# CliqueOfficial/zk-dcap-verifier

Hardware: AMD Instinct MI355X
Metric: proofs/hour sgx_dcap_verifier k=19 (create_proof on the GPU: commitments, lookups, grand products, NTTs, evaluate_h, evaluations, SHPLONK, host transcript; witness synthesis excluded) (higher is better)
Workload: dtype u32x8 (256-bit Montgomery integers)

## Files before the change

zk-dcap-verifier_amd/csrc/lookupperm.hip:

```cpp
#include "ctx.h"
#include <vector>

namespace zk {

constexpr uint32_t FS_T = 256, FS_E = 16, FS_TILE = FS_T * FS_E, FS_PAD = 258;

ZK_HD uint32_t fs_digit(uint2 k, uint32_t pass) { return ((pass < 4 ? k.x : k.y) >> (8 * (pass & 3))) & 255u; }

constexpr uint32_t XS_T = 256, XS_E = 8, XS_TILE = XS_T * XS_E;

ZK_HD int lp_cmp(const u256& a, const u256& b) {
    for (int i = 7; i >= 0; i--) {
        if (a.v[i] < b.v[i]) return -1;
        if (a.v[i] > b.v[i]) return 1;
    }
    return 0;
}
static uint32_t lp_scan_threads(uint32_t m) {
    uint32_t t = 64;
    while (t < 1024 && t * 8 < m) t <<= 1;
    return t;
}

struct LpbArgs {
    const void* const* cols;
    void* const* outs;
    const void* const* scols;
    const uint32_t* tabcol;
    uint32_t u, n, nb, S, C, nwg, nxs;
    void* canon; uint2* key_a; uint2* key_b; uint32_t* idx_a; uint32_t* idx_b;
    uint32_t* flags; uint32_t* ranks; uint32_t* leftover; uint32_t* ghist; uint32_t* xsums; uint32_t* scal;
    uint32_t* cscal;
    const uint32_t* shifts;
    const void* blind;
};
ZK_KERNEL void lpb_canon_kernel(LpbArgs a) {
    __shared__ uint32_t lor[8];
    const uint32_t s = blockIdx.y, i = blockIdx.x * blockDim.x + threadIdx.x;
    if (threadIdx.x < 8) lor[threadIdx.x] = 0;
    __syncthreads();
    if (i < a.u) {
        const u256 c = Fr::from_mont(load_u256(a.scols[s], i));
        store_u256(a.canon, (size_t)s * a.u + i, c);
#pragma unroll
        for (int w = 0; w < 8; w++) if (c.v[w] & ~lor[w]) atomicOr(&lor[w], c.v[w]);
    }
    __syncthreads();
    if (threadIdx.x < 8 && lor[threadIdx.x]) atomicOr(&a.cscal[s * 16 + threadIdx.x], lor[threadIdx.x]);
}
ZK_KERNEL void lpb_keys_kernel(LpbArgs a) {
    const uint32_t s = blockIdx.y, i = blockIdx.x * blockDim.x + threadIdx.x;
    if (i >= a.u) return;
    const uint32_t shift = a.shifts[s];
    const uint32_t* w = reinterpret_cast<const uint32_t*>(a.canon) + ((size_t)s * a.u + i) * 8;
    const uint32_t ws = shift >> 5, bs = shift & 31;
    uint32_t x[3];
#pragma unroll
    for (int j = 0; j < 3; j++) x[j] = ws + j < 8 ? w[ws + j] : 0u;
    uint2 k;
    k.x = bs ? (x[0] >> bs) | (x[1] << (32 - bs)) : x[0];
    k.y = bs ? (x[1] >> bs) | (x[2] << (32 - bs)) : x[1];
    a.key_a[(size_t)s * a.u + i] = k;
    a.idx_a[(size_t)s * a.u + i] = i;
}
ZK_KERNEL void lpb_hist_kernel(const uint2* keys, uint32_t u, uint32_t pass, uint32_t* ghist, uint32_t nwg) {
    __shared__ uint32_t lh[256];
    const uint32_t s = blockIdx.y, tid = threadIdx.x, base = blockIdx.x * FS_TILE;
    keys += (size_t)s * u;
    lh[tid] = 0;
    __syncthreads();
    for (uint32_t e = 0; e < FS_E; e++) {
        const uint32_t i = base + e * FS_T + tid;
        bool live = i < u;
        const uint32_t d = live ? fs_digit(keys[i], pass) : 0u;
#ifndef ZK_EMU
#pragma unroll
        for (int round = 0; round < 2; round++) {
            if (live) {
                const uint32_t lead = (uint32_t)__builtin_amdgcn_readfirstlane((int)d);
                const bool same = d == lead;
                const unsigned long long m = __ballot(same);
                if (same) {
                    if ((__lane_id() & 63u) == (uint32_t)__builtin_ctzll(m)) atomicAdd(&lh[lead], (uint32_t)__builtin_popcountll(m));
                    live = false;
                }
            }
        }
#endif
        if (live) atomicAdd(&lh[d], 1u);
    }
    __syncthreads();
    ghist[((size_t)s * nwg + blockIdx.x) * 256 + tid] = lh[tid];
}
ZK_KERNEL void lpb_offsets_kernel(uint32_t* ghist, uint32_t nwg) {
    __shared__ uint32_t scan[256];
    const uint32_t s = blockIdx.x, tid = threadIdx.x;
    uint32_t* h = ghist + (size_t)s * nwg * 256;
    uint32_t total = 0;
    for (uint32_t w = 0; w < nwg; w++) total += h[(size_t)w * 256 + tid];
    scan[tid] = total;
    __syncthreads();
    for (uint32_t d = 1; d < 256; d <<= 1) {
        const uint32_t add = tid >= d ? scan[tid - d] : 0;
        __syncthreads();
        scan[tid] += add;
        __syncthreads();
    }
    uint32_t run = scan[tid] - total;
    for (uint32_t w = 0; w < nwg; w++) {
        const uint32_t c = h[(size_t)w * 256 + tid];
        h[(size_t)w * 256 + tid] = run;
        run += c;
    }
}
ZK_KERNEL void lpb_scatter_kernel(const uint2* keys_in, const uint32_t* idx_in, uint2* keys_out, uint32_t* idx_out, uint32_t u, uint32_t pass,
                                  const uint32_t* gbase_all, uint32_t nwg) {
    __shared__ __attribute__((aligned(16))) uint16_t cnt[FS_T * FS_PAD];
    __shared__ uint32_t gbase[256];
    const uint32_t s = blockIdx.y, tid = threadIdx.x, wg = blockIdx.x, base = wg * FS_TILE;
    keys_in += (size_t)s * u; idx_in += (size_t)s * u; keys_out += (size_t)s * u; idx_out += (size_t)s * u;
    {
        uint4* c4 = reinterpret_cast<uint4*>(cnt);
        constexpr uint32_t n4 = FS_T * FS_PAD * 2 / 16;
        for (uint32_t q = tid; q < n4; q += FS_T) c4[q] = make_uint4(0, 0, 0, 0);
    }
    gbase[tid] = gbase_all[((size_t)s * nwg + wg) * 256 + tid];
    __syncthreads();
    uint2 k[FS_E];
    uint32_t v[FS_E];
    uint16_t rl[FS_E];
    const uint32_t lo = base + tid * FS_E;
#pragma unroll
    for (uint32_t e = 0; e < FS_E; e++) {
        const uint32_t i = lo + e;
        if (i < u) {
            k[e] = keys_in[i]; v[e] = idx_in[i];
            rl[e] = cnt[tid * FS_PAD + fs_digit(k[e], pass)]++;
        }
    }
    __syncthreads();
    {
        uint32_t run = 0;
        for (uint32_t t = 0; t < FS_T; t++) {
            const uint32_t c = cnt[t * FS_PAD + tid];
            cnt[t * FS_PAD + tid] = (uint16_t)run;
            run += c;
        }
    }
    __syncthreads();
#pragma unroll
    for (uint32_t e = 0; e < FS_E; e++) {
        const uint32_t i = lo + e;
        if (i < u) {
            const uint32_t d = fs_digit(k[e], pass);
            const uint32_t pos = gbase[d] + cnt[tid * FS_PAD + d] + rl[e];
            keys_out[pos] = k[e];
            idx_out[pos] = v[e];
        }
    }
}
ZK_KERNEL void lpb_check_kernel(LpbArgs a, const uint32_t* idx_sorted) {
    const uint32_t s = blockIdx.y, i = blockIdx.x * blockDim.x + threadIdx.x;
    if (i == 0 || i >= a.u || a.shifts[s] == 0) return;
    const uint32_t* canon = reinterpret_cast<const uint32_t*>(a.canon) + (size_t)s * a.u * 8;
    const uint32_t* idx = idx_sorted + (size_t)s * a.u;
    const uint32_t* x = canon + (size_t)idx[i - 1] * 8;
    const uint32_t* y = canon + (size_t)idx[i] * 8;
    for (int w = 7; w >= 0; w--) {
        if (x[w] < y[w]) return;
        if (x[w] > y[w]) { atomicAdd(&a.cscal[s * 16 + 8], 1u); return; }
    }
}
ZK_KERNEL void lpb_tiemask_kernel(LpbArgs a, const uint32_t* idx_sorted) {
    __shared__ uint32_t lor[8];
    const uint32_t s = blockIdx.y, i = blockIdx.x * blockDim.x + threadIdx.x;
    if (a.cscal[s * 16 + 8] == 0) return;
    if (threadIdx.x < 8) lor[threadIdx.x] = 0;
    __syncthreads();
    if (i > 0 && i < a.u) {
        const uint32_t shift = a.shifts[s];
        const uint32_t* canon = reinterpret_cast<const uint32_t*>(a.canon) + (size_t)s * a.u * 8;
        const uint32_t* idx = idx_sorted + (size_t)s * a.u;
        const uint32_t* x = canon + (size_t)idx[i - 1] * 8;
        const uint32_t* y = canon + (size_t)idx[i] * 8;
        uint32_t d[8], above = 0;
#pragma unroll
        for (int w = 0; w < 8; w++) {
            d[w] = x[w] ^ y[w];
            const uint32_t lo_bit = (uint32_t)w * 32;
            uint32_t in_window = lo_bit + 32 <= shift ? 0u : (lo_bit >= shift ? 0xffffffffu : (0xffffffffu << (shift - lo_bit)));
            above |= d[w] & in_window;
        }
        if (above == 0) {
#pragma unroll
            for (int w = 0; w < 8; w++) if (d[w] & ~lor[w]) atomicOr(&lor[w], d[w]);
        }
    }
    __syncthreads();
    if (threadIdx.x < 8 && lor[threadIdx.x]) atomicOr(&a.cscal[s * 16 + threadIdx.x], lor[threadIdx.x]);
}
ZK_KERNEL void lpb_rekey_kernel(LpbArgs a, const uint32_t* fcols, const uint32_t* fshift, const uint32_t* idx_in, uint2* key_out, uint32_t* idx_out) {
    const uint32_t f = blockIdx.y, i = blockIdx.x * blockDim.x + threadIdx.x;
    if (i >= a.u) return;
    const uint32_t c = fcols[f], shift = fshift[f];
    const uint32_t r = idx_in ? idx_in[(size_t)f * a.u + i] : i;
    const uint32_t* w = reinterpret_cast<const uint32_t*>(a.canon) + ((size_t)c * a.u + r) * 8;
    const uint32_t ws = shift >> 5, bs = shift & 31;
    uint32_t x[3];
#pragma unroll
    for (int j = 0; j < 3; j++) x[j] = ws + j < 8 ? w[ws + j] : 0u;
    uint2 k;
    k.x = bs ? (x[0] >> bs) | (x[1] << (32 - bs)) : x[0];
    k.y = bs ? (x[1] >> bs) | (x[2] << (32 - bs)) : x[1];
    key_out[(size_t)f * a.u + i] = k;
    idx_out[(size_t)f * a.u + i] = r;
}
ZK_KERNEL void lpb_mark_kernel(LpbArgs a, const uint32_t* idx_sorted) {
    const uint32_t l = blockIdx.y, i = blockIdx.x * blockDim.x + threadIdx.x, u = a.u;
    if (i >= u) return;
    const uint32_t tc = a.tabcol[l];
    const void* in_canon = (const char*)a.canon + (size_t)l * u * 32;
    const void* tab_canon = (const char*)a.canon + (size_t)tc * u * 32;
    const uint32_t* in_idx = idx_sorted + (size_t)l * u;
    const uint32_t* tab_idx = idx_sorted + (size_t)tc * u;
    uint32_t* repeated = a.flags + (size_t)(2 * l) * u;
    uint32_t* unconsumed = a.flags + (size_t)(2 * l + 1) * u;
    const u256 v = load_u256(in_canon, in_idx[i]);
    const bool first = i == 0 || lp_cmp(v, load_u256(in_canon, in_idx[i - 1])) != 0;
    repeated[i] = first ? 0u : 1u;
    if (!first) return;
    uint32_t lo = 0, hi = u;
    while (lo < hi) {
        const uint32_t mid = (lo + hi) >> 1;
        if (lp_cmp(load_u256(tab_canon, tab_idx[mid]), v) < 0) lo = mid + 1; else hi = mid;
    }
    if (lo >= u || lp_cmp(load_u256(tab_canon, tab_idx[lo]), v) != 0) { atomicAdd(&a.scal[l * 16 + 1], 1u); return; }
    unconsumed[lo] = 0;
}
ZK_KERNEL void lpb_fill_unconsumed_kernel(LpbArgs a) {
    const uint32_t l = blockIdx.y, i = blockIdx.x * blockDim.x + threadIdx.x;
    if (i < a.u) a.flags[(size_t)(2 * l + 1) * a.u + i] = 1u;
}
ZK_KERNEL void lpb_tile_sum_kernel(LpbArgs a) {
    __shared__ uint32_t part[XS_T];
    const uint32_t s = blockIdx.y, tid = threadIdx.x, base = blockIdx.x * XS_TILE;
    const uint32_t* v = a.ranks + (size_t)s * a.u;
    uint32_t sum = 0;
    for (uint32_t e = 0; e < XS_E; e++) { const uint32_t i = base + e * XS_T + tid; if (i < a.u) sum += v[i]; }
    part[tid] = sum;
    __syncthreads();
    for (uint32_t d = XS_T >> 1; d > 0; d >>= 1) { if (tid < d) part[tid] += part[tid + d]; __syncthreads(); }
    if (tid == 0) a.xsums[(size_t)s * a.nxs + blockIdx.x] = part[0];
}
ZK_KERNEL void lpb_sum_scan_kernel(LpbArgs a) {
    __shared__ uint32_t part[1024];
    const uint32_t s = blockIdx.x, T = blockDim.x, tid = threadIdx.x, m = a.nxs - 1;
    uint32_t* v = a.xsums + (size_t)s * a.nxs;
    const uint32_t per = (m + T - 1) / T;
    const uint32_t lo = tid * per < m ? tid * per : m, hi = lo + per < m ? lo + per : m;
    uint32_t sum = 0;
    for (uint32_t i = lo; i < hi; i++) sum += v[i];
    part[tid] = sum;
    __syncthreads();
    for (uint32_t d = 1; d < T; d <<= 1) {
        const uint32_t add = tid >= d ? part[tid - d] : 0;
        __syncthreads();
        part[tid] += add;
        __syncthreads();
    }
    uint32_t run = part[tid] - sum;
    for (uint32_t i = lo; i < hi; i++) { const uint32_t x = v[i]; v[i] = run; run += x; }
    if (tid == T - 1) a.scal[(s >> 1) * 16 + 2 + (s & 1)] = part[T - 1];
}
ZK_KERNEL void lpb_apply_kernel(LpbArgs a) {
    __shared__ uint32_t part[XS_T];
    const uint32_t s = blockIdx.y, tid = threadIdx.x, lo = blockIdx.x * XS_TILE + tid * XS_E, m = a.u;
    uint32_t* v = a.ranks + (size_t)s * a.u;
    uint32_t x[XS_E], sum = 0;
#pragma unroll
    for (uint32_t e = 0; e < XS_E; e++) { x[e] = lo + e < m ? v[lo + e] : 0u; sum += x[e]; }
    part[tid] = sum;
    __syncthreads();
    for (uint32_t d = 1; d < XS_T; d <<= 1) {
        const uint32_t add = tid >= d ? part[tid - d] : 0;
        __syncthreads();
        part[tid] += add;
        __syncthreads();
    }
    uint32_t run = a.xsums[(size_t)s * a.nxs + blockIdx.x] + part[tid] - sum;
#pragma unroll
    for (uint32_t e = 0; e < XS_E; e++) { if (lo + e < m) v[lo + e] = run; run += x[e]; }
}
ZK_KERNEL void lpb_compact_kernel(LpbArgs a) {
    const uint32_t l = blockIdx.y, t = blockIdx.x * blockDim.x + threadIdx.x;
    if (t < a.u && a.flags[(size_t)(2 * l + 1) * a.u + t]) a.leftover[(size_t)l * a.u + a.ranks[(size_t)(2 * l + 1) * a.u + t]] = t;
}
ZK_KERNEL void lpb_assemble_kernel(LpbArgs a, const uint32_t* idx_sorted) {
    const uint32_t l = blockIdx.y, i = blockIdx.x * blockDim.x + threadIdx.x, u = a.u;
    if (i >= a.n) return;
    void* out_in = a.outs[2 * l];
    void* out_tab = a.outs[2 * l + 1];
    if (i >= u) {
        store_u256(out_in, i, load_u256(a.blind, (size_t)(2 * l) * a.nb + (i - u)));
        store_u256(out_tab, i, load_u256(a.blind, (size_t)(2 * l + 1) * a.nb + (i - u)));
        return;
    }
    const uint32_t* in_idx = idx_sorted + (size_t)l * u;
    const uint32_t* tab_idx = idx_sorted + (size_t)a.tabcol[l] * u;
    const u256 v = load_u256(a.cols[2 * l], in_idx[i]);
    store_u256(out_in, i, v);
    if (!a.flags[(size_t)(2 * l) * u + i]) store_u256(out_tab, i, v);
    else {
        const uint32_t n_rep = a.scal[l * 16 + 2];
        store_u256(out_tab, i, load_u256(a.cols[2 * l + 1], tab_idx[a.leftover[(size_t)l * u + (n_rep - 1 - a.ranks[(size_t)(2 * l) * u + i])]]));
    }
}

int lookup_permute_batch(zk_ctx* ctx, const void* const* d_inputs, const void* const* d_tables, size_t count, uint32_t k, uint32_t blinding_factors,
                         const void* h_blind_inputs, const void* h_blind_tables, void* const* d_out_inputs, void* const* d_out_tables) {
    if (count == 0) return ZK_OK;
    if (!d_inputs || !d_tables || !d_out_inputs || !d_out_tables || !h_blind_inputs || !h_blind_tables)
        return ctx->fail(ZK_ERR_ARG, "zk_lookup_permute_batch_dev: null argument");
    if (k < 1 || k > 26 || count > 4096) return ctx->fail(ZK_ERR_ARG, "zk_lookup_permute_batch_dev: k = %u / count = %zu out of range", k, count);
    const uint32_t n = 1u << k, nb = blinding_factors + 1;
    if (nb >= n) return ctx->fail(ZK_ERR_ARG, "zk_lookup_permute_batch_dev: blinding_factors too large");
    for (size_t l = 0; l < count; l++)
        if (!d_inputs[l] || !d_tables[l] || !d_out_inputs[l] || !d_out_tables[l]) return ctx->fail(ZK_ERR_ARG, "zk_lookup_permute_batch_dev: null column %zu", l);
    const uint32_t u = n - nb, S = 2 * (uint32_t)count;
    std::vector<const void*> scols(d_inputs, d_inputs + count);
    std::vector<uint32_t> tabcol(count);
    for (size_t l = 0; l < count; l++) {
        size_t c = count;
        while (c < scols.size() && scols[c] != d_tables[l]) c++;
        if (c == scols.size()) scols.push_back(d_tables[l]);
        tabcol[l] = (uint32_t)c;
    }
    const uint32_t C = (uint32_t)scols.size();
    const uint32_t nwg = (u + FS_TILE - 1) / FS_TILE, nxs = (u + XS_TILE - 1) / XS_TILE + 1;
    size_t off = 0;
    auto take = [&](size_t bytes) { size_t o = off; off += (bytes + 255) & ~(size_t)255; return o; };
    const size_t o_canon = take((size_t)C * u * 32), o_blind = take((size_t)S * nb * 32), o_ka = take((size_t)C * u * 8), o_kb = take((size_t)C * u * 8),
                 o_ia = take((size_t)C * u * 4), o_ib = take((size_t)C * u * 4), o_fl = take((size_t)S * u * 4), o_rk = take((size_t)S * u * 4),
                 o_lo = take((size_t)count * u * 4), o_gh = take((size_t)C * nwg * 256 * 4), o_xs = take((size_t)S * nxs * 4), o_sc = take((size_t)count * 64),
                 o_cs = take((size_t)C * 64), o_sh = take((size_t)C * 4), o_tc = take((size_t)count * 4), o_cp = take((size_t)S * sizeof(void*)),
                 o_op = take((size_t)S * sizeof(void*)), o_sp = take((size_t)C * sizeof(void*));
    ZK_HIP(ctx->ws_tmp.ensure(off + 256));
    char* base = (char*)ctx->ws_tmp.p;
    hipStream_t st = ctx->stream;
    std::vector<const void*> cols(S);
    std::vector<void*> outs(S);
    std::vector<unsigned char> blind((size_t)S * nb * 32);
    for (size_t l = 0; l < count; l++) {
        cols[2 * l] = d_inputs[l]; cols[2 * l + 1] = d_tables[l];
        outs[2 * l] = d_out_inputs[l]; outs[2 * l + 1] = d_out_tables[l];
        memcpy(&blind[(2 * l) * (size_t)nb * 32], (const char*)h_blind_inputs + l * (size_t)nb * 32, (size_t)nb * 32);
        memcpy(&blind[(2 * l + 1) * (size_t)nb * 32], (const char*)h_blind_tables + l * (size_t)nb * 32, (size_t)nb * 32);
    }
    ZK_HIP(hipMemcpyAsync(base + o_cp, cols.data(), S * sizeof(void*), hipMemcpyHostToDevice, st));
    ZK_HIP(hipMemcpyAsync(base + o_op, outs.data(), S * sizeof(void*), hipMemcpyHostToDevice, st));
    ZK_HIP(hipMemcpyAsync(base + o_sp, scols.data(), C * sizeof(void*), hipMemcpyHostToDevice, st));
    ZK_HIP(hipMemcpyAsync(base + o_tc, tabcol.data(), count * 4, hipMemcpyHostToDevice, st));
    ZK_HIP(hipMemcpyAsync(base + o_blind, blind.data(), blind.size(), hipMemcpyHostToDevice, st));
    ZK_HIP(hipMemsetAsync(base + o_sc, 0, count * 64, st));
    ZK_HIP(hipMemsetAsync(base + o_cs, 0, (size_t)C * 64, st));
    LpbArgs a;
    memset(&a, 0, sizeof a);
    a.cols = (const void* const*)(base + o_cp); a.outs = (void* const*)(base + o_op); a.scols = (const void* const*)(base + o_sp);
    a.tabcol = (const uint32_t*)(base + o_tc);
    a.u = u; a.n = n; a.nb = nb; a.S = S; a.C = C; a.nwg = nwg; a.nxs = nxs;
    a.canon = base + o_canon; a.key_a = (uint2*)(base + o_ka); a.key_b = (uint2*)(base + o_kb); a.idx_a = (uint32_t*)(base + o_ia); a.idx_b = (uint32_t*)(base + o_ib);
    a.flags = (uint32_t*)(base + o_fl); a.ranks = (uint32_t*)(base + o_rk); a.leftover = (uint32_t*)(base + o_lo); a.ghist = (uint32_t*)(base + o_gh);
    a.xsums = (uint32_t*)(base + o_xs); a.scal = (uint32_t*)(base + o_sc); a.cscal = (uint32_t*)(base + o_cs); a.shifts = (const uint32_t*)(base + o_sh);
    a.blind = base + o_blind;
    const int blk = ctx->tune.vec_block;
    const uint32_t g = (u + blk - 1) / blk;
    ZK_LAUNCH(lpb_canon_kernel, dim3(g, C), blk, 0, st, a);
    ZK_CHECK_LAUNCH();
    std::vector<uint32_t> sc((size_t)count * 16), csc((size_t)C * 16);
    ZK_HIP(hipMemcpyAsync(csc.data(), a.cscal, (size_t)C * 64, hipMemcpyDeviceToHost, st));
    ZK_HIP(hipStreamSynchronize(st));
    std::vector<uint32_t> shifts(C);
    uint32_t max_bits = 1;
    bool any_shift = false;
    for (uint32_t c = 0; c < C; c++) {
        const uint32_t* om = &csc[(size_t)c * 16];
        uint32_t nbits = 1;
        for (int wd = 7; wd >= 0; wd--)
            if (om[wd]) { uint32_t top = 31; while (!((om[wd] >> top) & 1)) top--; nbits = (uint32_t)wd * 32 + top + 1; break; }
        shifts[c] = nbits > 64 ? nbits - 64 : 0;
        any_shift |= shifts[c] != 0;
        max_bits = std::max(max_bits, std::min(nbits, 64u));
    }
    ZK_HIP(hipMemcpyAsync(base + o_sh, shifts.data(), (size_t)C * 4, hipMemcpyHostToDevice, st));
    uint32_t* sorted = a.idx_a;
    const bool use_order_check = any_shift;

    auto compact_sort = [&](const std::vector<uint32_t>& fcols, const std::vector<std::vector<uint32_t>>& stage_shift, const std::vector<uint32_t>& stage_bits) -> int {
        const uint32_t Fn = (uint32_t)fcols.size();
        if (!Fn) return ZK_OK;
        const size_t per = (size_t)Fn * u;
        size_t o2 = 0;
        auto take2 = [&](size_t bytes) { size_t o = o2; o2 += (bytes + 255) & ~(size_t)255; return o; };
        const size_t q_ka = take2(per * 8), q_kb = take2(per * 8), q_ia = take2(per * 4), q_ib = take2(per * 4), q_gh = take2((size_t)Fn * nwg * 256 * 4),
                     q_fc = take2((size_t)Fn * 4), q_fs = take2((size_t)Fn * 4 * stage_shift.size());
        ZK_HIP(ctx->ws_mid.ensure(o2 + 256));
        char* b2 = (char*)ctx->ws_mid.p;
        uint2 *rk_in = (uint2*)(b2 + q_ka), *rk_out = (uint2*)(b2 + q_kb);
        uint32_t *ri_in = (uint32_t*)(b2 + q_ia), *ri_out = (uint32_t*)(b2 + q_ib), *rgh = (uint32_t*)(b2 + q_gh);
        ZK_HIP(hipMemcpyAsync(b2 + q_fc, fcols.data(), (size_t)Fn * 4, hipMemcpyHostToDevice, st));
        for (size_t t = 0; t < stage_shift.size(); t++)
            ZK_HIP(hipMemcpyAsync(b2 + q_fs + t * Fn * 4, stage_shift[t].data(), (size_t)Fn * 4, hipMemcpyHostToDevice, st));
        const uint32_t* order = nullptr;
        for (size_t t = 0; t < stage_shift.size(); t++) {
            ZK_LAUNCH(lpb_rekey_kernel, dim3(g, Fn), blk, 0, st, a, (const uint32_t*)(b2 + q_fc), (const uint32_t*)(b2 + q_fs + t * Fn * 4), order, rk_in, ri_in);
            ZK_CHECK_LAUNCH();
            const uint32_t ps = (stage_bits[t] + 7) / 8;
            for (uint32_t p = 0; p < ps; p++) {
                ZK_LAUNCH(lpb_hist_kernel, dim3(nwg, Fn), FS_T, 0, st, (const uint2*)rk_in, u, p, rgh, nwg);
                ZK_CHECK_LAUNCH();
                ZK_LAUNCH(lpb_offsets_kernel, Fn, 256, 0, st, rgh, nwg);
                ZK_CHECK_LAUNCH();
                ZK_LAUNCH(lpb_scatter_kernel, dim3(nwg, Fn), FS_T, 0, st, (const uint2*)rk_in, (const uint32_t*)ri_in, rk_out, ri_out, u, p, (const uint32_t*)rgh, nwg);
                ZK_CHECK_LAUNCH();
                std::swap(rk_in, rk_out);
                std::swap(ri_in, ri_out);
            }
            std::swap(rk_in, rk_out);
            std::swap(ri_in, ri_out);
            order = ri_out;
        }
        for (uint32_t f = 0; f < Fn; f++)
            ZK_HIP(hipMemcpyAsync(sorted + (size_t)fcols[f] * u, order + (size_t)f * u, (size_t)u * 4, hipMemcpyDeviceToDevice, st));
        return ZK_OK;
    };
    auto low_stages = [&](const std::vector<uint32_t>& fcols, const std::vector<uint32_t>& lo_bit, const std::vector<uint32_t>& hi_bit,
                          std::vector<std::vector<uint32_t>>& stage_shift, std::vector<uint32_t>& stage_bits) {
        const uint32_t Fn = (uint32_t)fcols.size();
        uint32_t n_low = 0;
        for (uint32_t f = 0; f < Fn; f++) if (lo_bit[f] < 256) n_low = std::max(n_low, (hi_bit[f] - lo_bit[f]) / 64 + 1);
        for (uint32_t t = 0; t < n_low; t++) {
            std::vector<uint32_t> sh(Fn);
            uint32_t bits = 1;
            for (uint32_t f = 0; f < Fn; f++) {
                const uint32_t st_lo = lo_bit[f] == 256 ? 256 : lo_bit[f] + 64 * t;
                if (st_lo > hi_bit[f] || st_lo >= 256) { sh[f] = 255; continue; }
                sh[f] = st_lo;
                bits = std::max(bits, std::min(64u, hi_bit[f] - st_lo + 1));
            }
            stage_shift.push_back(sh); stage_bits.push_back(bits);
        }
        std::vector<uint32_t> sh(Fn);
        for (uint32_t f = 0; f < Fn; f++) sh[f] = shifts[fcols[f]];
        stage_shift.push_back(sh); stage_bits.push_back(max_bits);
    };
    auto tie_ranges = [&](const std::vector<uint32_t>& cols_, std::vector<uint32_t>& lo_bit, std::vector<uint32_t>& hi_bit) -> int {
        for (uint32_t c : cols_) ZK_HIP(hipMemsetAsync((char*)a.cscal + (size_t)c * 64, 0, 32, st));
        ZK_LAUNCH(lpb_tiemask_kernel, dim3(g, C), blk, 0, st, a, (const uint32_t*)sorted); ZK_CHECK_LAUNCH();
        ZK_HIP(hipMemcpyAsync(csc.data(), a.cscal, (size_t)C * 64, hipMemcpyDeviceToHost, st));
// ... 92 lines not shown
```

zk-dcap-verifier_amd/csrc/mockprover.hip:

```cpp
#include "ctx.h"
#include "quotient.h"
#include <algorithm>
#include <atomic>
#include <list>
#include <random>
#include <string>

namespace zk {
int quotient_program_load(zk_ctx* ctx, const void* blob, size_t len, uint64_t* prog);
int quotient_program_release(zk_ctx* ctx, uint64_t prog);

namespace {
constexpr uint32_t MP_T = 256, MP_E = 8, MP_TILE = MP_T * MP_E, MP_WAVES = MP_T / 64;
constexpr uint32_t MP_LOCAL = 2 * MP_T;

__device__ inline uint64_t mp_ballot(bool p, uint32_t* lds) {
#ifdef ZK_EMU
    const uint32_t tid = threadIdx.x;
    lds[tid] = p ? 1u : 0u;
    __syncthreads();
    uint64_t m = 0;
    for (uint32_t l = 0; l < 64; l++) if (lds[(tid & ~63u) + l]) m |= 1ull << l;
    __syncthreads();
    return m;
#else
    (void)lds;
    return __ballot(p);
#endif
}

ZK_KERNEL void ZK_LAUNCH_BOUNDS(256) mp_count_kernel(const uint8_t* flags, uint64_t count, uint32_t* tile_counts) {
    __shared__ uint32_t bl[MP_T];
    __shared__ uint32_t wc[MP_WAVES];
    const uint32_t tid = threadIdx.x, wave = tid >> 6, lane = tid & 63u;
    const uint64_t base = (uint64_t)blockIdx.x * MP_TILE;
    uint32_t mine = 0;
    for (uint32_t e = 0; e < MP_E; e++) {
        const uint64_t i = base + (uint64_t)e * MP_T + tid;
        mine += (uint32_t)__builtin_popcountll(mp_ballot(i < count && flags[i], bl));
    }
    if (lane == 0) wc[wave] = mine;
    __syncthreads();
    if (tid == 0) {
        uint32_t s = 0;
        for (uint32_t w = 0; w < MP_WAVES; w++) s += wc[w];
        tile_counts[blockIdx.x] = s;
    }
}
ZK_KERNEL void ZK_LAUNCH_BOUNDS(256) mp_scan_kernel(uint32_t* counts, uint32_t n_tiles) {
    __shared__ uint32_t s[MP_T];
    const uint32_t tid = threadIdx.x, per = (n_tiles + MP_T - 1) / MP_T;
    const uint32_t lo = tid * per < n_tiles ? tid * per : n_tiles, hi = lo + per < n_tiles ? lo + per : n_tiles;
    uint32_t sum = 0;
    for (uint32_t i = lo; i < hi; i++) sum += counts[i];
    s[tid] = sum;
    __syncthreads();
    for (uint32_t d = 1; d < MP_T; d <<= 1) {
        const uint32_t v = tid >= d ? s[tid - d] : 0u;
        __syncthreads();
        s[tid] += v;
        __syncthreads();
    }
    uint32_t run = s[tid] - sum;
    for (uint32_t i = lo; i < hi; i++) { const uint32_t c = counts[i]; counts[i] = run; run += c; }
    if (tid == MP_T - 1) counts[n_tiles] = s[MP_T - 1];
}
ZK_KERNEL void ZK_LAUNCH_BOUNDS(256) mp_scatter_kernel(const uint8_t* flags, uint64_t count, const uint32_t* tile_offsets, uint32_t* out) {
    __shared__ uint32_t bl[MP_T];
    __shared__ uint32_t wc[MP_E][MP_WAVES];
    const uint32_t tid = threadIdx.x, wave = tid >> 6, lane = tid & 63u;
    const uint64_t base = (uint64_t)blockIdx.x * MP_TILE;
    uint64_t masks[MP_E];
    for (uint32_t e = 0; e < MP_E; e++) {
        const uint64_t i = base + (uint64_t)e * MP_T + tid;
        masks[e] = mp_ballot(i < count && flags[i], bl);
        if (lane == 0) wc[e][wave] = (uint32_t)__builtin_popcountll(masks[e]);
    }
    __syncthreads();
    uint32_t pos = tile_offsets[blockIdx.x];
    for (uint32_t e = 0; e < MP_E; e++) {
        uint32_t before = 0;
        for (uint32_t w = 0; w < wave; w++) before += wc[e][w];
        if ((masks[e] >> lane) & 1ull)
            out[pos + before + (uint32_t)__builtin_popcountll(masks[e] & ((1ull << lane) - 1ull))] = (uint32_t)(base + (uint64_t)e * MP_T + tid);
        for (uint32_t w = 0; w < MP_WAVES; w++) pos += wc[e][w];
    }
}

ZK_KERNEL void mp_nonzero_kernel(const void* vals, uint32_t u, uint8_t* flags) {
    const uint32_t i = blockIdx.x * blockDim.x + threadIdx.x;
    if (i < u) flags[i] = Fr::is_zero(load_u256(vals, i)) ? 0 : 1;
}

ZK_HD bool mp_less(const u256& a, const u256& b) {
    for (int w = 7; w >= 0; w--)
        if (a.v[w] != b.v[w]) return a.v[w] < b.v[w];
    return false;
}
ZK_KERNEL void mp_table_init_kernel(const void* src, uint32_t u, uint32_t n, void* dst) {
    const uint32_t i = blockIdx.x * blockDim.x + threadIdx.x;
    if (i >= n) return;
    u256 v;
    if (i < u) v = load_u256(src, i);
    else for (int w = 0; w < 8; w++) v.v[w] = 0xffffffffu;
    store_u256(dst, i, v);
}
ZK_KERNEL void mp_bitonic_step_kernel(void* v, uint32_t n, uint32_t size, uint32_t dist) {
    const uint32_t t = blockIdx.x * blockDim.x + threadIdx.x;
    if (t >= n / 2) return;
    const uint32_t lo = ((t & ~(dist - 1u)) << 1) | (t & (dist - 1u)), hi = lo | dist;
    const u256 a = load_u256(v, lo), b = load_u256(v, hi);
    if (mp_less(b, a) == ((lo & size) == 0)) { store_u256(v, lo, b); store_u256(v, hi, a); }
}
ZK_KERNEL void ZK_LAUNCH_BOUNDS(256) mp_bitonic_local_kernel(void* v, uint32_t size_lo, uint32_t size_hi) {
    __shared__ uint4 s[2 * MP_LOCAL];
    const uint32_t tid = threadIdx.x, T = blockDim.x, base = blockIdx.x * 2 * T;
    const uint4* g = reinterpret_cast<const uint4*>(v) + 2 * (size_t)base;
    for (uint32_t j = tid; j < 4 * T; j += T) s[j] = g[j];
    __syncthreads();
    for (uint32_t size = size_lo; size <= size_hi; size <<= 1) {
        for (uint32_t dist = size / 2 < T ? size / 2 : T; dist > 0; dist >>= 1) {
            const uint32_t lo = ((tid & ~(dist - 1u)) << 1) | (tid & (dist - 1u)), hi = lo | dist;
            u256 a, b;
            const uint4 a0 = s[2 * lo], a1 = s[2 * lo + 1], b0 = s[2 * hi], b1 = s[2 * hi + 1];
            a.v[0] = a0.x; a.v[1] = a0.y; a.v[2] = a0.z; a.v[3] = a0.w; a.v[4] = a1.x; a.v[5] = a1.y; a.v[6] = a1.z; a.v[7] = a1.w;
            b.v[0] = b0.x; b.v[1] = b0.y; b.v[2] = b0.z; b.v[3] = b0.w; b.v[4] = b1.x; b.v[5] = b1.y; b.v[6] = b1.z; b.v[7] = b1.w;
            if (mp_less(b, a) == (((base + lo) & size) == 0)) { s[2 * lo] = b0; s[2 * lo + 1] = b1; s[2 * hi] = a0; s[2 * hi + 1] = a1; }
            __syncthreads();
        }
    }
    uint4* o = reinterpret_cast<uint4*>(v) + 2 * (size_t)base;
    for (uint32_t j = tid; j < 4 * T; j += T) o[j] = s[j];
}
ZK_KERNEL void mp_search_kernel(const void* in, const void* sorted, uint32_t k, uint32_t u, uint8_t* flags) {
    const uint32_t r = blockIdx.x * blockDim.x + threadIdx.x;
    if (r >= u) return;
    const u256 x = load_u256(in, r);
    uint32_t pos = 0;
    for (uint32_t b = (1u << k) >> 1; b; b >>= 1)
        if (mp_less(load_u256(sorted, pos + b - 1), x)) pos += b;
    flags[r] = Fr::eq(load_u256(sorted, pos), x) ? 0 : 1;
}
ZK_KERNEL void mp_copy_kernel(const void* const* cols, const uint32_t* map_c, const uint32_t* map_r, uint32_t n_cols, uint32_t k, uint8_t* flags, uint32_t* bad) {
    const uint64_t e = (uint64_t)blockIdx.x * blockDim.x + threadIdx.x;
    if (e >= ((uint64_t)n_cols << k)) return;
    const uint32_t j = (uint32_t)(e >> k), row = (uint32_t)e & ((1u << k) - 1u), cj = map_c[e], rj = map_r[e];
    uint8_t f = 0;
    if (cj >= n_cols || rj >= (1u << k)) atomicOr(bad, 1u);
    else if (cj != j || rj != row) f = Fr::eq(Fr::normalize(load_u256(cols[j], row)), Fr::normalize(load_u256(cols[cj], rj))) ? 0 : 1;
    flags[e] = f;
}

ZK_KERNEL void ZK_LAUNCH_BOUNDS(256) mp_edge_flag_kernel(const uint32_t* map_c, const uint32_t* map_r, uint32_t n_cols, uint32_t k, uint8_t* flags, uint32_t* bad) {
    const uint64_t cells = (uint64_t)n_cols << k, stride = (uint64_t)gridDim.x * blockDim.x;
    for (uint64_t e = (uint64_t)blockIdx.x * blockDim.x + threadIdx.x; e < cells; e += stride) {
        const uint32_t cj = map_c[e], rj = map_r[e];
        uint8_t f = 0;
        if (cj >= n_cols || rj >= (1u << k)) atomicOr(bad, 1u);
        else f = (((uint64_t)cj << k) | rj) != e ? 1 : 0;
        flags[e] = f;
    }
}
ZK_KERNEL void ZK_LAUNCH_BOUNDS(256) mp_edge_gather_kernel(const uint32_t* moved, uint32_t n_edges, const uint32_t* map_c, const uint32_t* map_r, uint32_t k, uint2* edges) {
    const uint32_t stride = gridDim.x * blockDim.x;
    for (uint64_t i = blockIdx.x * blockDim.x + threadIdx.x; i < n_edges; i += stride) {
        const uint32_t c = moved[i];
        edges[i] = make_uint2(c, (map_c[c] << k) | map_r[c]);
    }
}
ZK_KERNEL void ZK_LAUNCH_BOUNDS(256) mp_copy_edges_kernel(const void* const* cols, const uint2* edges, uint32_t n_edges, uint32_t k, uint8_t* flags) {
    const uint32_t stride = gridDim.x * blockDim.x, mask = (1u << k) - 1u;
    for (uint64_t i = blockIdx.x * blockDim.x + threadIdx.x; i < n_edges; i += stride) {
        const uint2 e = edges[i];
        flags[i] = Fr::eq(Fr::normalize(load_u256(cols[e.x >> k], e.x & mask)), Fr::normalize(load_u256(cols[e.y >> k], e.y & mask))) ? 0 : 1;
    }
}
ZK_KERNEL void ZK_LAUNCH_BOUNDS(256) mp_edge_pick_kernel(const uint32_t* picked, uint32_t count, const uint2* edges, uint2* out) {
    const uint32_t stride = gridDim.x * blockDim.x;
    for (uint64_t i = blockIdx.x * blockDim.x + threadIdx.x; i < count; i += stride) out[i] = edges[picked[i]];
}

struct MpMem {
    std::list<DevTmp> held;
    void* get(size_t bytes) {
        held.emplace_back();
        if (hipMalloc(&held.back().p, bytes ? bytes : 32) != hipSuccess) { held.back().p = nullptr; return nullptr; }
        return held.back().p;
    }
};

int mp_oom(zk_ctx* ctx, const char* fn) { return ctx->fail(ZK_ERR_HIP, "%s: device allocation failed", fn); }

int mp_compact(zk_ctx* ctx, const char* fn, const uint8_t* d_flags, uint64_t count, uint32_t* cnt, DevBuf& list, uint32_t* total) {
    const uint32_t tiles = (uint32_t)((count + MP_TILE - 1) / MP_TILE);
    *total = 0;
    if (!tiles) return ZK_OK;
    ZK_LAUNCH(mp_count_kernel, tiles, MP_T, 0, ctx->stream, d_flags, count, cnt);
    ZK_CHECK_LAUNCH();
    ZK_LAUNCH(mp_scan_kernel, 1, MP_T, 0, ctx->stream, cnt, tiles);
    ZK_CHECK_LAUNCH();
    ZK_HIP(hipMemcpyAsync(total, cnt + tiles, 4, hipMemcpyDeviceToHost, ctx->stream));
    ZK_HIP(hipStreamSynchronize(ctx->stream));
    if (!*total) return ZK_OK;
    if (list.ensure((size_t)*total * 4) != hipSuccess) return mp_oom(ctx, fn);
    ZK_LAUNCH(mp_scatter_kernel, tiles, MP_T, 0, ctx->stream, d_flags, count, (const uint32_t*)cnt, (uint32_t*)list.p);
    ZK_CHECK_LAUNCH();
    return ZK_OK;
}

int mp_sort(zk_ctx* ctx, void* d_v, uint32_t k) {
    const uint32_t n = 1u << k, T = std::min<uint32_t>(MP_T, n / 2), L = 2 * T;
    ZK_LAUNCH(mp_bitonic_local_kernel, n / L, T, 0, ctx->stream, d_v, 2u, L);
    ZK_CHECK_LAUNCH();
    for (uint32_t size = 2 * L; size <= n; size <<= 1) {
        for (uint32_t dist = size / 2; dist >= L; dist >>= 1) {
            ZK_LAUNCH(mp_bitonic_step_kernel, (n / 2 + 255) / 256, 256, 0, ctx->stream, d_v, n, size, dist);
            ZK_CHECK_LAUNCH();
        }
        ZK_LAUNCH(mp_bitonic_local_kernel, n / L, T, 0, ctx->stream, d_v, size, size);
        ZK_CHECK_LAUNCH();
    }
    return ZK_OK;
}

u256 mp_random_nonzero(std::mt19937_64& g) {
    for (;;) {
        u256 x;
        for (int i = 0; i < 8; i += 2) { const uint64_t w = g(); x.v[i] = (uint32_t)w; x.v[i + 1] = (uint32_t)(w >> 32); }
        x.v[7] &= 0x3fffffffu;
        x = Fr::reduce_once(x);
        if (!Fr::is_zero(x)) return x;
    }
}

struct MpTimer {
    EvTimer t;
    MpTimer(zk_ctx* ctx, const char* label) : t(ctx, label) {}
    void done() { t.stop(); t.resolve(); }
};

}

struct MockPlan {
    bool copy_edges;
    bool resident_tables;
};
constexpr MockPlan MP_ONE_SHOT{false, false};
constexpr MockPlan MP_SESSION{true, true};

struct MockSession {
    zk_ctx* ctx;
    MockPlan plan = MP_SESSION;
    uint32_t k = 0, n = 0, u = 0, F = 0, A = 0, I = 0, L = 0, M = 0, n_challenges = 0, n_polys = 0, words = 0, n_edges = 0, n_programs = 0;
    uint64_t cells = 0;
    size_t bytes = 0;
    std::vector<void*> owned;
    std::vector<uint64_t> progs;
    std::vector<uint32_t> perm_cols;
    std::vector<const void*> fx;
    std::vector<void*> inst, adv_stage;
    void *zero_col = nullptr, *work = nullptr, *d_cp = nullptr;
    uint2* edges = nullptr;
    const uint32_t *map_c = nullptr, *map_r = nullptr;
    uint32_t *d_mc = nullptr, *d_mr = nullptr, *d_bad = nullptr;
    uint8_t* flags = nullptr;
    uint32_t* tile_counts = nullptr;
    DevBuf copy_list, gate_list, lookup_list, gate_bits, picked;
    uint64_t gate_prog = 0;
    struct Table { uint64_t prog; bool resident; void* sorted; };
    std::vector<Table> tables;
    std::vector<uint64_t> input_prog;
    std::vector<uint32_t> table_of;
    const u256 one = Fr::one();
    u256 theta;
    std::mt19937_64 rng;

    explicit MockSession(zk_ctx* c) : ctx(c) {}
    MockSession(const MockSession&) = delete;
    MockSession& operator=(const MockSession&) = delete;
    void* get(size_t b) {
        void* p = nullptr;
        if (hipMalloc(&p, b ? b : 32) != hipSuccess) return nullptr;
        owned.push_back(p);
        bytes += b ? b : 32;
        return p;
    }
    ~MockSession() {
        (void)hipSetDevice(ctx->device);
        for (void* p : owned) (void)hipFree(p);
        for (DevBuf* b : {&copy_list, &gate_list, &lookup_list, &gate_bits, &picked}) b->release();
        for (uint64_t h : progs) (void)quotient_program_release(ctx, h);
    }
};

namespace {
std::atomic<uint64_t> g_mock_session_id{1};
enum class MpChallenges { Refused, Given, Evaluator };

uint32_t mp_edge_grid(zk_ctx* ctx, uint64_t count) {
    const uint64_t want = (count + MP_T - 1) / MP_T, cap = ctx->tune.mock_edge_wgs > 0 ? (uint64_t)ctx->tune.mock_edge_wgs : 1;
    return (uint32_t)std::max<uint64_t>(1, std::min(want, cap));
}
bool mp_reads_fixed_only(const QuotProgram& P) {
    if (P.uses_xpow || P.part_hi || P.part_lo) return false;
    for (const uint4& ins : P.code)
        for (uint32_t src : {ins.y, ins.z, ins.w}) {
            const uint32_t kind = src >> 28, pay = src & 0x0fffffffu;
            if (kind == K_COL) { const uint32_t c = pay >> 8; if (c < P.col_fixed || c >= P.col_fixed + P.n_fixed) return false; }
            else if (kind == K_CONST) { if (pay >= P.c_chal && pay < P.c_chal + P.n_challenges) return false; }
            else if (kind != K_SLOT && kind != K_ACC && kind != K_NONE) return false;
        }
    return true;
}
MockSession* mp_session(zk_ctx* ctx, uint64_t mp, const char* fn) {
    auto it = ctx->mock_sessions.find(mp);
    if (it == ctx->mock_sessions.end()) { (void)ctx->fail(ZK_ERR_ARG, "%s: unknown handle %llu (closed, or opened on another context)", fn, (unsigned long long)mp); return nullptr; }
    return it->second.get();
}

zk_mock_witness mp_witness_of(const zk_mock_desc* d, const void* challenges, uint32_t n_challenges) {
    zk_mock_witness w;
    ZK_STRUCT_INIT(w);
    w.advice_values = d->advice_values; w.instances = d->instances; w.instance_lens = d->instance_lens; w.values_on_device = d->values_on_device;
    w.challenges = challenges; w.n_challenges = n_challenges;
    return w;
}
int mp_witness_args(zk_ctx* ctx, const char* fn, uint32_t A, uint32_t I, uint32_t n, const zk_mock_witness& w) {
    if (A && !w.advice_values) return ctx->fail(ZK_ERR_ARG, "%s: missing advice column array", fn);
    for (uint32_t i = 0; i < A; i++) if (!w.advice_values[i]) return ctx->fail(ZK_ERR_ARG, "%s: advice column %u is NULL", fn, i);
    for (uint32_t c = 0; c < I; c++) {
        const uint32_t len = w.instance_lens ? w.instance_lens[c] : 0;
        if (len > n || (len && (!w.instances || !w.instances[c]))) return ctx->fail(ZK_ERR_ARG, "%s: instance column %u: %u values", fn, c, len);
    }
    return ZK_OK;
}

int mp_validate(zk_ctx* ctx, const zk_mock_desc* d, const char* fn, MpChallenges rule, uint32_t* n_challenges, bool witness) {
    if (!d) return ctx->fail(ZK_ERR_ARG, "%s: null descriptor", fn);
    if (d->struct_size != sizeof(zk_mock_desc))
        return ctx->fail(ZK_ERR_ARG, "%s: zk_mock_desc.struct_size %u, expected %zu (ABI version %u)", fn, d->struct_size, sizeof(zk_mock_desc), ZK_ABI_VERSION);
    const uint32_t k = d->k, F = d->n_fixed, A = d->n_advice, I = d->n_instance, L = d->n_lookups, M = d->n_perm_columns;
    if (k < 2 || k > 26 || (uint64_t)d->blinding_factors + 1 >= (1ull << k)) return ctx->fail(ZK_ERR_ARG, "%s: k = %u with %u blinding factors", fn, k, d->blinding_factors);
    const uint32_t n = 1u << k, u = n - d->blinding_factors - 1;
    if ((F && !d->fixed_values) || (L && (!d->lookup_input_zkq1 || !d->lookup_input_zkq1_len || !d->lookup_table_zkq1 || !d->lookup_table_zkq1_len)) ||
        (M && (!d->perm_columns || !d->perm_map_column || !d->perm_map_row)) || !d->evaluator_zkq1)
        return ctx->fail(ZK_ERR_ARG, "%s: missing column / program / mapping array", fn);
    for (uint32_t i = 0; i < F; i++) if (!d->fixed_values[i]) return ctx->fail(ZK_ERR_ARG, "%s: fixed column %u is NULL", fn, i);
    if (witness) {
        const int rc = mp_witness_args(ctx, fn, A, I, n, mp_witness_of(d, nullptr, 0));
        if (rc) return rc;
    }
    for (uint32_t j = 0; j < M; j++) {
        const uint32_t ty = d->perm_columns[2 * j], ix = d->perm_columns[2 * j + 1];
        if (ty > 2 || ix >= (ty == 0 ? A : ty == 1 ? F : I)) return ctx->fail(ZK_ERR_ARG, "%s: permutation column %u = (%u, %u) out of range", fn, j, ty, ix);
    }
    if (((uint64_t)M << k) >= (1ull << 32) || (uint64_t)L * u >= (1ull << 32)) return ctx->fail(ZK_ERR_LIMIT, "%s: more than 2^32 cells to check in one pass", fn);
    auto header = [&](const void* blob, size_t len, bool evaluator, const char* what, uint32_t i) -> int {
        if (!blob || len < 48 || (len & 3)) return ctx->fail(ZK_ERR_ARG, "%s: bad %s blob %u", fn, what, i);
        uint32_t w[7];
        memcpy(w, blob, sizeof w);
        if (w[0] != 0x31514B5Au) return ctx->fail(ZK_ERR_PROGRAM, "%s: %s blob %u: bad magic", fn, what, i);
        switch (rule) {
        case MpChallenges::Refused:
            if (w[6]) return ctx->fail(ZK_ERR_PROGRAM, "%s: %s blob %u declares %u challenges (their values go to zk_mock_prover_verify_phased)", fn, what, i, w[6]);
            break;
        case MpChallenges::Given:
            if (w[6] != *n_challenges) return ctx->fail(ZK_ERR_ARG, "zk_mock_prover_verify_phased: %s blob %u declares %u challenges, the caller passed %u", what, i, w[6], *n_challenges);
            break;
        case MpChallenges::Evaluator:
            if (evaluator) *n_challenges = w[6];
            if (w[6] != *n_challenges) return ctx->fail(ZK_ERR_ARG, "%s: %s blob %u declares %u challenges, the evaluator %u", fn, what, i, w[6], *n_challenges);
            if (w[6] > ZK_MAX_CHALLENGES) return ctx->fail(ZK_ERR_LIMIT, "%s: %u challenges, the quotient interpreter's constant bank is sized for %u", fn, w[6], ZK_MAX_CHALLENGES);
            break;
        }
        if (w[1] != k || (!evaluator && w[2] != k)) return ctx->fail(ZK_ERR_ARG, "%s: %s blob %u is for k = %u / extended_k = %u, not k = %u", fn, what, i, w[1], w[2], k);
        if (w[3] != F || w[4] != A || w[5] != I)
            return ctx->fail(ZK_ERR_ARG, "%s: %s blob %u has %u / %u / %u fixed / advice / instance columns, the descriptor %u / %u / %u", fn, what, i, w[3], w[4], w[5], F, A, I);
        return ZK_OK;
// ... 370 lines not shown
```

Baseline: 73930.

## Replace per-thread LDS digit histograms with wave-level ballot match in radix scatter

The radix-sort scatter kernel used to keep a padded 256x258 uint16 per-thread counter table in LDS, which had to be zeroed and then prefix-scanned serially over 256 threads. It now builds per-wave digit counters by matching equal digits across a wave with eight ballots, so one leader lane updates the counter and the other lanes take their rank from a popcount. Elements are read in a wave-strided layout to keep the sort stable with the per-wave offsets. This shrinks LDS use and the scan work, and should allow higher occupancy, at the cost of about nine ballots per element plus wave-level fences. The ballot helper also moves into a shared header.

```diff
diff --git a/zk-dcap-verifier_amd/csrc/lookupperm.hip b/zk-dcap-verifier_amd/csrc/lookupperm.hip
--- a/zk-dcap-verifier_amd/csrc/lookupperm.hip
+++ b/zk-dcap-verifier_amd/csrc/lookupperm.hip
@@ -1,9 +1,10 @@
 #include "ctx.h"
+#include "wave.h"
 #include <vector>
 
 namespace zk {
 
-constexpr uint32_t FS_T = 256, FS_E = 16, FS_TILE = FS_T * FS_E, FS_PAD = 258;
+constexpr uint32_t FS_T = 256, FS_E = 16, FS_TILE = FS_T * FS_E, FS_WAVES = FS_T / 64, FS_WROWS = FS_TILE / FS_WAVES;
 
 ZK_HD uint32_t fs_digit(uint2 k, uint32_t pass) { return ((pass < 4 ? k.x : k.y) >> (8 * (pass & 3))) & 255u; }
 
@@ -113,47 +114,65 @@
         run += c;
     }
 }
-ZK_KERNEL void lpb_scatter_kernel(const uint2* keys_in, const uint32_t* idx_in, uint2* keys_out, uint32_t* idx_out, uint32_t u, uint32_t pass,
-                                  const uint32_t* gbase_all, uint32_t nwg) {
-    __shared__ __attribute__((aligned(16))) uint16_t cnt[FS_T * FS_PAD];
+ZK_KERNEL void ZK_LAUNCH_BOUNDS(256) lpb_scatter_kernel(const uint2* keys_in, const uint32_t* idx_in, uint2* keys_out, uint32_t* idx_out, uint32_t u, uint32_t pass,
+                                                         const uint32_t* gbase_all, uint32_t nwg) {
+    __shared__ uint32_t wcnt[FS_WAVES][256];
     __shared__ uint32_t gbase[256];
-    const uint32_t s = blockIdx.y, tid = threadIdx.x, wg = blockIdx.x, base = wg * FS_TILE;
+    __shared__ uint32_t bl[FS_T];
+    const uint32_t s = blockIdx.y, tid = threadIdx.x, wave = tid >> 6, lane = tid & 63u, wg = blockIdx.x;
     keys_in += (size_t)s * u; idx_in += (size_t)s * u; keys_out += (size_t)s * u; idx_out += (size_t)s * u;
-    {
-        uint4* c4 = reinterpret_cast<uint4*>(cnt);
-        constexpr uint32_t n4 = FS_T * FS_PAD * 2 / 16;
-        for (uint32_t q = tid; q < n4; q += FS_T) c4[q] = make_uint4(0, 0, 0, 0);
-    }
+#pragma unroll
+    for (uint32_t w = 0; w < FS_WAVES; w++) wcnt[w][tid] = 0;
     gbase[tid] = gbase_all[((size_t)s * nwg + wg) * 256 + tid];
     __syncthreads();
     uint2 k[FS_E];
     uint32_t v[FS_E];
-    uint16_t rl[FS_E];
-    const uint32_t lo = base + tid * FS_E;
+    uint32_t rd[FS_E];
+    const uint32_t lo = wg * FS_TILE + wave * FS_WROWS + lane;
+    const uint64_t below = (1ull << lane) - 1ull;
 #pragma unroll
     for (uint32_t e = 0; e < FS_E; e++) {
-        const uint32_t i = lo + e;
-        if (i < u) {
-            k[e] = keys_in[i]; v[e] = idx_in[i];
-            rl[e] = cnt[tid * FS_PAD + fs_digit(k[e], pass)]++;
-        }
+        const uint32_t i = lo + 64 * e;
+        k[e] = i < u ? keys_in[i] : make_uint2(0, 0);
+        v[e] = i < u ? idx_in[i] : 0u;
+    }
+#pragma unroll
+    for (uint32_t e = 0; e < FS_E; e++) {
+        const bool live = lo + 64 * e < u;
+        const uint32_t d = fs_digit(k[e], pass);
+        const uint64_t lv = wave_ballot(live, bl);
+        uint32_t plo = (uint32_t)lv, phi = (uint32_t)(lv >> 32);
+#pragma unroll
+        for (uint32_t b = 0; b < 8; b++) {
+            const uint64_t m = wave_ballot((d >> b) & 1u, bl);
+            const uint32_t x = 0u - ((d >> b) & 1u);
+            plo &= ~((uint32_t)m ^ x);
+            phi &= ~((uint32_t)(m >> 32) ^ x);
+        }
+        const uint64_t peers = (uint64_t)phi << 32 | plo;
+        const uint32_t lower = (uint32_t)__builtin_popcountll(peers & below);
+        const uint32_t old = wcnt[wave][d];
+        wave_lds_order();
+        if (live && lower == 0) wcnt[wave][d] = old + (uint32_t)__builtin_popcountll(peers);
+        wave_lds_order();
+        rd[e] = d << 16 | (old + lower);
     }
     __syncthreads();
     {
         uint32_t run = 0;
-        for (uint32_t t = 0; t < FS_T; t++) {
-            const uint32_t c = cnt[t * FS_PAD + tid];
-            cnt[t * FS_PAD + tid] = (uint16_t)run;
+#pragma unroll
+        for (uint32_t w = 0; w < FS_WAVES; w++) {
+            const uint32_t c = wcnt[w][tid];
+            wcnt[w][tid] = run;
             run += c;
         }
     }
     __syncthreads();
 #pragma unroll
     for (uint32_t e = 0; e < FS_E; e++) {
-        const uint32_t i = lo + e;
-        if (i < u) {
-            const uint32_t d = fs_digit(k[e], pass);
-            const uint32_t pos = gbase[d] + cnt[tid * FS_PAD + d] + rl[e];
+        if (lo + 64 * e < u) {
+            const uint32_t d = rd[e] >> 16;
+            const uint32_t pos = gbase[d] + wcnt[wave][d] + (rd[e] & 0xffffu);
             keys_out[pos] = k[e];
             idx_out[pos] = v[e];
         }
diff --git a/zk-dcap-verifier_amd/csrc/mockprover.hip b/zk-dcap-verifier_amd/csrc/mockprover.hip
--- a/zk-dcap-verifier_amd/csrc/mockprover.hip
+++ b/zk-dcap-verifier_amd/csrc/mockprover.hip
@@ -1,5 +1,6 @@
 #include "ctx.h"
 #include "quotient.h"
+#include "wave.h"
 #include <algorithm>
 #include <atomic>
 #include <list>
@@ -13,21 +14,6 @@
 namespace {
 constexpr uint32_t MP_T = 256, MP_E = 8, MP_TILE = MP_T * MP_E, MP_WAVES = MP_T / 64;
 constexpr uint32_t MP_LOCAL = 2 * MP_T;
-
-__device__ inline uint64_t mp_ballot(bool p, uint32_t* lds) {
-#ifdef ZK_EMU
-    const uint32_t tid = threadIdx.x;
-    lds[tid] = p ? 1u : 0u;
-    __syncthreads();
-    uint64_t m = 0;
-    for (uint32_t l = 0; l < 64; l++) if (lds[(tid & ~63u) + l]) m |= 1ull << l;
-    __syncthreads();
-    return m;
-#else
-    (void)lds;
-    return __ballot(p);
-#endif
-}
 
 ZK_KERNEL void ZK_LAUNCH_BOUNDS(256) mp_count_kernel(const uint8_t* flags, uint64_t count, uint32_t* tile_counts) {
     __shared__ uint32_t bl[MP_T];
@@ -37,7 +23,7 @@
     uint32_t mine = 0;
     for (uint32_t e = 0; e < MP_E; e++) {
         const uint64_t i = base + (uint64_t)e * MP_T + tid;
-        mine += (uint32_t)__builtin_popcountll(mp_ballot(i < count && flags[i], bl));
+        mine += (uint32_t)__builtin_popcountll(wave_ballot(i < count && flags[i], bl));
     }
     if (lane == 0) wc[wave] = mine;
     __syncthreads();
@@ -73,7 +59,7 @@
     uint64_t masks[MP_E];
     for (uint32_t e = 0; e < MP_E; e++) {
         const uint64_t i = base + (uint64_t)e * MP_T + tid;
-        masks[e] = mp_ballot(i < count && flags[i], bl);
+        masks[e] = wave_ballot(i < count && flags[i], bl);
         if (lane == 0) wc[e][wave] = (uint32_t)__builtin_popcountll(masks[e]);
     }
     __syncthreads();
diff --git a/zk-dcap-verifier_amd/csrc/wave.h b/zk-dcap-verifier_amd/csrc/wave.h
--- /dev/null
+++ b/zk-dcap-verifier_amd/csrc/wave.h
@@ -0,0 +1,31 @@
+#pragma once
+#include "rt.h"
+
+namespace zk {
+
+__device__ inline uint64_t wave_ballot(bool p, uint32_t* lds) {
+#ifdef ZK_EMU
+    const uint32_t tid = threadIdx.x;
+    lds[tid] = p ? 1u : 0u;
+    __syncthreads();
+    uint64_t m = 0;
+    for (uint32_t l = 0; l < 64; l++) if (lds[(tid & ~63u) + l]) m |= 1ull << l;
+    __syncthreads();
+    return m;
+#else
+    (void)lds;
+    return __ballot(p);
+#endif
+}
+
+__device__ inline void wave_lds_order() {
+#ifdef ZK_EMU
+    __syncthreads();
+#else
+    __builtin_amdgcn_fence(__ATOMIC_RELEASE, "wavefront");
+    __builtin_amdgcn_wave_barrier();
+    __builtin_amdgcn_fence(__ATOMIC_ACQUIRE, "wavefront");
+#endif
+}
+
+}
```

Measured after the change: 74600 (median of 5 runs). Within noise of the previous version (+0.9%).
